# jhuggins/viabel

Measured on AMD Instinct MI355X. Metric: ELBO-gradient evals/sec (D=1024, N_mc=4096), higher is better.
Workload: dtype f64

## Files before the change

viabel_amd/csrc/vb_fullrank.hip:

```cpp
#include "vb_gemm_f64.h"
#include "vb_fit.h"

namespace vb {

constexpr double kLog2PiFr = 1.8378770664093454835606594728112;

__device__ __forceinline__ double fr_wave_sum(double x) {
#pragma unroll
  for (int off = 32; off > 0; off >>= 1) x += __shfl_down(x, off, 64);
  return x;
}

__device__ __forceinline__ double fr_block_sum(double x, double* sh) {
  x = fr_wave_sum(x);
  const int lane = threadIdx.x & 63, wave = threadIdx.x >> 6;
  __syncthreads();
  if (lane == 0) sh[wave] = x;
  __syncthreads();
  return (sh[0] + sh[1]) + (sh[2] + sh[3]);
}

__global__ void __launch_bounds__(256) fr_unpack_kernel(const double* __restrict__ theta, int d,
                                                        int64_t ldl, double* __restrict__ Lt,
                                                        double* __restrict__ mu, double* __restrict__ copy = nullptr) {
// ... 282 lines not shown
        if (roww) g[i] *= rw[i];
        if (square) g[i] *= g[i];
        if (!in) g[i] = (fr_d2){0.0, 0.0}, z[i] = (fr_d2){0.0, 0.0};
        if (!ok1) g[i].y = 0.0, z[i].y = 0.0;
        if (Gscaled && in) *reinterpret_cast<fr_d2*>(Gscaled + r * ldz + col) = g[i] * rs[i];
        s += g[i];
        if (fmode == 1) f = fma(hiv.x * g[i].x, g[i].x, fma(hiv.y * g[i].y, g[i].y, f));
        if (fmode == 2) f = fma(0.5 * z[i].x, g[i].x, fma(0.5 * z[i].y, g[i].y, f));
        if (fmode == 3) f = fma(-0.5 * scal * z[i].x, z[i].x, fma(-0.5 * scal * z[i].y, z[i].y, f));
      }
    }
  }
  cs[q][c] = s;
  __syncthreads();
  if (q == 0 && ok0) {
    const fr_d2 tot = (cs[0][c] + cs[1][c]) + (cs[2][c] + cs[3][c]);
    colpart[(int64_t)blockIdx.y * ldz + col] = tot.x;
    if (ok1) colpart[(int64_t)blockIdx.y * ldz + col + 1] = tot.y;
  }
  f = fr_block_sum(f, sh);
  if (threadIdx.x == 0) fpart[(int64_t)blockIdx.y * gridDim.x + blockIdx.x] = f;
}

__global__ void __launch_bounds__(256) fr_fold_msum_kernel(const double* __restrict__ Mpart, int msplits, int64_t slab,
                                                           int d, int64_t ldz, int k_split, int bm_rows,
                                                           double* __restrict__ Mout, int nb_b,
                                                           const double* __restrict__ P, int64_t ldp,
                                                           const double* __restrict__ mu,
                                                           const double* __restrict__ mean, double* __restrict__ b) {
  if ((int)blockIdx.x >= nb_b) {
    const int bpr = (int)((ldz / 2 + 255) / 256);
    const int blk = (int)blockIdx.x - nb_b, r = blk / bpr;
    const int cp = (blk - r * bpr) * 256 + (int)threadIdx.x;
    if (2 * cp >= ldz) return;
    const int64_t idx = (int64_t)r * ldz + 2 * cp;
    const int z0 = (r / bm_rows * bm_rows) / kGemmBK * kGemmBK / k_split;
    fr_d2 s = (fr_d2){0.0, 0.0};
    for (int zb = z0; zb < msplits; zb += 4) {
      fr_d2 v[4];
#pragma unroll
      for (int u = 0; u < 4; ++u)
        v[u] = *reinterpret_cast<const fr_d2*>(Mpart + (zb + u < msplits ? zb + u : msplits - 1) * slab + idx);
      s = zb == z0 ? v[0] : s + v[0];
#pragma unroll
      for (int u = 1; u < 4; ++u)
        if (zb + u < msplits) s += v[u];
    }
    *reinterpret_cast<fr_d2*>(Mout + idx) = s;
    return;
  }
  __shared__ fr_d2 part[64][4];
  const int p = threadIdx.x & 3, kg = threadIdx.x >> 2;
  const int col = (int)blockIdx.x * 8 + 2 * p;
  const int colc = col < d ? col : 0;
  const int kper = (d + 63) / 64;
  const int k0 = kg * kper, k1 = k0 + kper < d ? k0 + kper : d;
  fr_d2 s = (fr_d2){0.0, 0.0};
  for (int kb = k0; kb < k1; kb += 16) {
    fr_d2 v[16];
    double c[16];
#pragma unroll
    for (int u = 0; u < 16; ++u) {
      const int k = kb + u < k1 ? kb + u : k1 - 1;
      v[u] = *reinterpret_cast<const fr_d2*>(P + (int64_t)k * ldp + colc);
      c[u] = mu[k] - mean[k];
    }
#pragma unroll
    for (int u = 0; u < 16; ++u)
      if (kb + u < k1) s += v[u] * c[u];
  }
  part[kg][p] = s;
  __syncthreads();
  if (kg == 0) {
    fr_d2 tot = part[0][p];
#pragma unroll
    for (int q = 1; q < 64; ++q) tot += part[q][p];
    if (col < d) b[col] = tot.x;
    if (col + 1 < d) b[col + 1] = tot.y;
  }
}

static int fr_fold_splits(int d) {
  const int s = d / (16 * kGemmBK);
  return s < 1 ? 1 : (s > 8 ? 8 : s);
}

__global__ void __launch_bounds__(256) fr_fold_ssum_kernel(const double* __restrict__ Spart, int gsplits, int64_t slab, int d,
                                                           int64_t ldl, const double* __restrict__ colpart, int64_t ldz,
                                                           const double* __restrict__ M, const double* __restrict__ b,
                                                           double n_rows, int nb_cs, int nb_s,
                                                           double* __restrict__ S, double* __restrict__ svec,
                                                           double* __restrict__ csg) {
  if ((int)blockIdx.x < nb_cs) {
    __shared__ fr_d2 part[64][4];
    const int p = threadIdx.x & 3, kg = threadIdx.x >> 2;
    const int col = (int)blockIdx.x * 8 + 2 * p;
    const int colc = col < d ? col : 0;
    const int kper = (d + 63) / 64;
    const int k0 = kg * kper, k1 = k0 + kper < d ? k0 + kper : d;
    fr_d2 acc = (fr_d2){0.0, 0.0};
    for (int kb = k0; kb < k1; kb += 16) {
      fr_d2 v[16];
      double c[16];
#pragma unroll
      for (int u = 0; u < 16; ++u) {
        const int k = kb + u < k1 ? kb + u : k1 - 1;
        v[u] = *reinterpret_cast<const fr_d2*>(M + (int64_t)k * ldz + colc);
        c[u] = colpart[k];
      }
      for (int z = 1; z < gsplits; ++z)
#pragma unroll
        for (int u = 0; u < 16; ++u) c[u] += colpart[(int64_t)z * ldz + (kb + u < k1 ? kb + u : k1 - 1)];
#pragma unroll
      for (int u = 0; u < 16; ++u)
        if (kb + u < k1) acc += v[u] * c[u];
    }
    part[kg][p] = acc;
    __syncthreads();
    if (kg == 0) {
      fr_d2 tot = part[0][p];
#pragma unroll
      for (int q = 1; q < 64; ++q) tot += part[q][p];
      if (col < d) csg[col] = -tot.x - n_rows * b[col];
      if (col + 1 < d) csg[col + 1] = -tot.y - n_rows * b[col + 1];
    }
    return;
  }
  if ((int)blockIdx.x < nb_cs + nb_s) {
    const int k = ((int)blockIdx.x - nb_cs) * 256 + (int)threadIdx.x;
    if (k >= ldz) return;
    double s = 0.0;
    if (k < d) {
      s = colpart[k];
      for (int z = 1; z < gsplits; ++z) s += colpart[(int64_t)z * ldz + k];
    }
    svec[k] = s;
    return;
  }
  int bi = 0, bj = (int)blockIdx.x - nb_cs - nb_s;
  while (bj > bi) bj -= ++bi;
  __shared__ double tile[32][33];
  const int tx = threadIdx.x & 31, ty = threadIdx.x >> 5;
  const int i0 = bi * 32, j0 = bj * 32;
  double v[4];
  int64_t idx[4];
#pragma unroll
  for (int q = 0; q < 4; ++q) {
// ... 790 lines not shown
#endif
  *tiles2_out = (unsigned)n_p2;
  return VB_OK;
}


enum FrDense {
  kDenseNoG,
  kDenseCallerG,
  kDensePersistent,
  kDenseChain
};

struct FrRoute {
  bool mvt = false, pd = false, glm = false, source = false, overlap = false;
  int n_cu = 0;
  int64_t n = 0, d = 0, ldl = 0, ldz = 0, ldr = 0, slab = 0, pslab = 0, np = 0, glm_part = 0;
  int D = 0, n_rb = 0, cs_gx = 0, n_fpart = 0;
  int tri1 = 0, tri3 = 0;
  int splits = 1;
  int kparts = 1;
  unsigned sum_blocks = 0;
  bool fold_shape = false;
  int msplits = 1;
  bool fold = false;
  int csplits = 1;
  int cfgc = 0;
  int fz_mode = 0;
  FrDense dense = kDenseChain;
  bool model_ksplit = false;
  bool caller_z = false;
  bool fused_sums = false;
  bool diag_f = false;
  bool cs_only = false;
  bool g_prescaled = false;
  bool scale_rows_w = false;
  bool two_passes = false;
  bool colpass = false;
  bool colpass_keeps_f = false;
  int fmode = 0;
  bool grad_colsums = false;
  bool grad_launch = true;
  int cfg3 = 0;
  bool f_per_tile = false;
};

static FrRoute fr_route(const vb_ctx* ctx, const ModelDev& m, int64_t n, int64_t d, bool mvt, bool pd, bool row_scaled,
// ... 27 lines not shown
  if (r.splits > max_splits) r.splits = max_splits;
  if (r.splits < 1) r.splits = 1;
  r.n_rb = (int)((n + 127) / 128);
  r.cs_gx = (D + 127) / 128;
  r.glm_part = r.glm ? gemm_max_blocks(n, m.n_data) : 0;
  r.ldr = r.glm ? round_up(m.n_data, 16) : 0;
  r.n_fpart = funnel ? (int)((n + 3) / 4) : r.source ? (int)n : r.n_rb * r.cs_gx + (int)r.glm_part;

  const bool sums_in_gemms = !mvt && !wm.roww && !row_scaled && n % kGemmBK == 0 && gemm_uses_dma(s1) &&
                             (int64_t)r.splits <= r.n_rb;
  r.fused_sums = gauss_full && sums_in_gemms;
  r.diag_f = gauss_diag && sums_in_gemms;

  if (!row_scaled && !pd && !gauss_diag) {
    const long tiles64 = gemm_count_blocks(s1, 64, 64);
    if (tiles64 < 2L * n_cu && D >= 48 * kGemmBK) r.kparts = (int)((2L * n_cu + tiles64 - 1) / tiles64);
    if (r.kparts > 4) r.kparts = 4;
    while (r.kparts > 1 && (D % (kGemmBK * r.kparts) != 0 || D / r.kparts < 16 * kGemmBK)) --r.kparts;
    if ((int64_t)r.kparts * r.pslab > (int64_t)(r.splits + 1) * r.slab) r.kparts = 1;
  }
  r.sum_blocks = (unsigned)((r.pslab / 2 + 255) / 256);

  r.fold_shape = !mvt && gauss_full && !pd && d >= VB_FR_FOLD_MIN_D && n >= (int64_t)VB_FR_FOLD_MIN_ROWS_PER_D * d;
  r.msplits = fr_fold_splits(D);
  r.fold = r.fold_shape && r.fused_sums && r.kparts == 1 && !wm.z_ready && !wm.g_ready && n >= d + 2;

  r.fz_mode = ctx->fr_fused_mode;
  if (r.fz_mode < 0) {
    const char* e = getenv("VB_FR_FUSED");
    r.fz_mode = e ? atoi(e) : 0;
  }
  if (!(r.fused_sums && r.kparts == 1 && n % 128 == 0 && D % 64 == 0 && (int64_t)n * r.ldz * 8 < ((int64_t)1 << 31)))
    r.fz_mode = 0;
  if ((r.fz_mode != 2 && r.fz_mode != 3) || pd || r.fold || wm.g_ready) r.fz_mode = 0;
  r.dense = r.fold ? kDenseNoG : wm.g_ready ? kDenseCallerG : r.fz_mode >= 2 ? kDensePersistent : kDenseChain;
  r.model_ksplit = r.kparts > 1 && r.fused_sums;
  r.caller_z = wm.z_ready != nullptr && (funnel || r.source || r.glm);

  r.g_prescaled = funnel && wm.roww != nullptr;
  r.scale_rows_w = wm.roww != nullptr && !r.g_prescaled;
  r.cs_only = r.diag_f || (!r.fused_sums && !mvt && (funnel || r.source) && (!wm.roww || r.g_prescaled) && !row_scaled &&
                           n % kGemmBK == 0 && gemm_uses_dma(s3) && (int64_t)r.splits <= r.n_rb);
  const bool f_from_pass = !(funnel || r.source);
  r.colpass = !r.fused_sums && !r.cs_only;
  r.two_passes = pd && r.colpass && f_from_pass;
  r.colpass_keeps_f = f_from_pass && !r.two_passes;
  r.fmode = gauss_diag ? 1 : r.glm ? 3 : (gauss_full && !wm.g_ready) ? 2 : 0;

  r.grad_launch = r.fz_mode != 3;
  r.grad_colsums = r.fused_sums || r.cs_only;
  if (r.grad_launch && r.grad_colsums && gemm_count_blocks(s3, 128, 64) * r.splits * 100 >= 190L * n_cu) r.cfg3 = 2;
  r.f_per_tile = r.fused_sums || r.diag_f;
  if (r.fold) {
    r.csplits = fr_fold_csplits(D, n_cu, r.splits + 1);
    const GemmArgs sc = gemm_product(nullptr, 0, nullptr, 0, D, D, D, 2);
    if (gemm_count_blocks(sc, 64, 64) * r.csplits <= 4L * n_cu) r.cfgc = 4;
    else r.cfgc = gemm_count_blocks(sc, 128, 64) * r.csplits * 100 >= 190L * n_cu ? 2 : 3;
  }
  return r;
}

struct FrBufs {
  const double* E = nullptr;
  int64_t lde = 0;
  double *mu = nullptr, *Lt = nullptr;
  double *Z = nullptr, *G = nullptr, *Cpart = nullptr, *colpart = nullptr, *fpart = nullptr;
  double* Rm = nullptr;
  double *Mpart = nullptr, *bvec = nullptr;
  double *Sg = nullptr, *svec = nullptr, *csg = nullptr;
  double *Xa = nullptr, *T = nullptr, *sq = nullptr;
  FrSums S;
};

static int fr_carve(vb_ctx* ctx, const FrRoute& r, const NoiseSlot& ns, int set, FrBufs* out) {
  const int64_t n = r.n, ldz = r.ldz, slab = r.slab;
  int64_t off = 0;
  auto carve = [&off](int64_t doubles) {
    const int64_t o = off;
    off += round_up(doubles, 16);
    return o;
  };
  const int64_t o_mu = carve(ldz), o_lt = carve(slab), o_z = carve(n * ldz), o_g = carve(n * ldz),
                o_cpart = carve((int64_t)(r.splits + 1) * slab), o_col = carve((int64_t)(r.n_rb + 1) * ldz),
                o_fpart = carve((int64_t)r.n_fpart + (int64_t)r.n_rb * r.cs_gx + gemm_max_blocks(n, r.D) + (n * ldz) / 512 + 1),
                o_r = carve(r.glm ? n * r.ldr : 0);
  const int64_t o_mpart = r.fold_shape ? carve((int64_t)(r.msplits + 1) * slab) : 0, o_bvec = r.fold_shape ? carve(ldz) : 0;
  const int64_t o_xa = r.pd ? carve(slab) : 0, o_t = r.pd ? carve(slab) : 0, o_m2 = r.pd ? carve(256) : 0;
  FrBufs b;
  b.S.off_col = 16;
  b.S.off_c = 16 + ldz;
  b.S.len = 16 + ldz + (r.mvt ? slab : round_up(r.np, 16));
  const int64_t o_sums = carve(b.S.len * (r.overlap ? 2 : 1));
  VB_TRY(ensure(ctx, ctx->fr_work, (size_t)off * sizeof(double)));
  double* base = (double*)ctx->fr_work.ptr;
  b.E = (const double*)ns.buf.ptr;
  b.lde = ns.ld;
  b.mu = base + o_mu, b.Lt = base + o_lt, b.Z = base + o_z, b.G = base + o_g, b.Cpart = base + o_cpart;
  b.colpart = base + o_col, b.fpart = base + o_fpart, b.Rm = base + o_r;
  b.Mpart = base + o_mpart, b.bvec = base + o_bvec;
  if (r.fold) b.Sg = b.G, b.svec = b.G + slab, b.csg = b.G + slab + ldz;
  b.Xa = base + o_xa, b.T = base + o_t, b.sq = base + o_m2;
  b.S.sums = base + o_sums + (int64_t)set * b.S.len;
  *out = b;
  return VB_OK;
}

static int fr_stream_plan(vb_ctx* ctx, const FrRoute& r, int* set) {
  Pipeline& P = ctx->pipe;
  hipStream_t st = ctx->stream;
  *set = 0;
  if (r.overlap) {
    VB_TRY(pipe_init(ctx));
    *set = (int)(ctx->fr_seq++ & 1);
    if (P.fin_valid[*set]) VB_HIP(ctx, hipStreamWaitEvent(st, P.ev_fin[*set], 0));
  } else if (P.post_pending) {
    VB_HIP(ctx, hipStreamWaitEvent(st, P.ev_fin[P.last_set], 0));
    P.post_pending = false;
  }
  return VB_OK;
}

static int fr_prepare_mvt(vb_ctx* ctx, const FrRoute& r, const FrBufs& b, const double* mu_dev, const double* root_dev) {
// ... 69 lines not shown
static int fr_model_funnel(vb_ctx* ctx, const FrRoute& r, const FrBufs& b, const ModelDev& m, const double* Z,
                           const double* roww) {
  hipLaunchKernelGGL(fr_funnel_kernel, dim3((unsigned)((r.n + 3) / 4)), dim3(256), 0, ctx->stream, Z, b.G, r.ldz, r.n, r.D, m,
                     b.fpart, roww);
  return VB_OK;
}

static int fr_model_source(vb_ctx* ctx, const FrRoute& r, const FrBufs& b, const double* Z) {
  return model_rows_enqueue(ctx, ctx->stream, Z, r.ldz, r.n, r.D, b.G, r.ldz, b.fpart);
}

static int fr_model_glm(vb_ctx* ctx, const FrRoute& r, const FrBufs& b, const ModelDev& m, const double* Z) {
  hipStream_t st = ctx->stream;
  double* part = b.fpart + (int64_t)r.n_rb * r.cs_gx;
  VB_HIP(ctx, hipMemsetAsync(part, 0, (size_t)r.glm_part * sizeof(double), st));
  const GemmArgs gh = gemm_product(Z, r.ldz, m.p1, m.ldq, (int)r.n, (int)m.n_data, r.D, 0);
  gemm_f64_launch<true>(st, gh, 1, r.n_cu, EpiGlm{b.Rm, r.ldr, m.p2, part, m.link, m.aux});
  VB_HIP(ctx, hipGetLastError());
  return glm_grad_enqueue(ctx, st, m, b.Rm, r.ldr, Z, b.G, r.ldz, r.n, r.D);
}

static int fr_model_folded(vb_ctx* ctx, const FrRoute& r, const FrBufs& b, const ModelDev& m) {
  hipStream_t st = ctx->stream;
  const int D = r.D, msplits = r.msplits;
  double* Mres = msplits > 1 ? b.Mpart + (int64_t)msplits * r.slab : b.Mpart;
  const GemmArgs gm = gemm_product(b.Lt, r.ldl, m.p1, m.ldp, D, D, D, 4);
  gemm_f64_launch<true>(st, gm, msplits, r.n_cu, EpiSplitSlab{b.Mpart, r.ldz, r.slab}, 4);
  const int ks = (int)round_up((D + msplits - 1) / msplits, kGemmBK);
  const int nb_sum = msplits > 1 ? D * (int)((r.ldz / 2 + 255) / 256) : 0, nb_b = (D + 7) / 8;
  hipLaunchKernelGGL(fr_fold_msum_kernel, dim3((unsigned)(nb_sum + nb_b)), dim3(256), 0, st, (const double*)b.Mpart, msplits,
                     r.slab, D, r.ldz, ks, 64, Mres, nb_b, m.p1, (int64_t)m.ldp, (const double*)b.mu, m.p0, b.bvec);
  VB_HIP(ctx, hipGetLastError());
  return VB_OK;
}

static int fr_grad_folded(vb_ctx* ctx, const FrRoute& r, const FrBufs& b, unsigned* tiles3) {
  hipStream_t st = ctx->stream;
  const int D = r.D;
  const double* M = r.msplits > 1 ? b.Mpart + (int64_t)r.msplits * r.slab : b.Mpart;
  GemmArgs gs = gemm_product(b.E, b.lde, b.E, b.lde, D, D, (int)r.n, 2);
  prof_events(ctx, &gs.ev0, &gs.ev1, 1, VB_PROF_FR_GRAD_GEMM);
  if (r.cfg3 == 2) VB_TRY(tri2_tile_map(ctx, D, 128, 64, &gs.tile_map, &gs.tile_blocks));
  gemm_f64_launch<false>(st, gs, r.splits, r.n_cu, EpiSplitSlabCs{b.Cpart, r.ldl, r.slab, b.colpart, r.ldz}, r.cfg3);
  VB_HIP(ctx, hipGetLastError());
  const int nb_cs = (D + 7) / 8, nb_s = (int)((r.ldz + 255) / 256), tiles = (D + 31) / 32;
  hipLaunchKernelGGL(fr_fold_ssum_kernel, dim3((unsigned)(nb_cs + nb_s + tiles * (tiles + 1) / 2)), dim3(256), 0, st,
                     (const double*)b.Cpart, r.splits, r.slab, D, r.ldl, (const double*)b.colpart, r.ldz, M,
                     (const double*)b.bvec, (double)r.n, nb_cs, nb_s, b.Sg, b.svec, b.csg);
  VB_HIP(ctx, hipGetLastError());
  GemmArgs gc = gemm_product(M, r.ldz, b.Sg, r.ldl, D, D, D, 2);
  if (r.cfgc == 2) VB_TRY(tri2_tile_map(ctx, D, 128, 64, &gc.tile_map, &gc.tile_blocks));
  *tiles3 = gemm_f64_launch<false>(st, gc, r.csplits, r.n_cu,
                                   EpiFoldSlabF{b.Cpart, r.ldl, r.slab, b.bvec, b.svec, b.Lt, r.ldl, b.fpart}, r.cfgc);
  VB_HIP(ctx, hipGetLastError());
  return VB_OK;
}

static int fr_model_gauss_full(vb_ctx* ctx, const FrRoute& r, const FrBufs& b, const ModelDev& m, const double* row_scale,
                               const double* g_ready, double** G, unsigned* tiles2) {
  hipStream_t st = ctx->stream;
  const int D = r.D;
  *G = b.G;
  GemmArgs g2 = gemm_product(b.Z, r.ldz, m.p1, m.ldp, (int)r.n, D, D, 0);
  switch (r.dense) {
    case kDenseNoG:
      return fr_model_folded(ctx, r, b, m);
    case kDenseCallerG:
      *G = const_cast<double*>(g_ready);
      return VB_OK;
    case kDensePersistent: {
      const GemmArgs g1 = gemm_product(b.E, b.lde, b.Lt, r.ldl, (int)r.n, D, D, r.tri1);
// ... 24 lines not shown
                      double* fpart, const double* row_scale) {
  hipLaunchKernelGGL(fr_colsum_kernel, dim3((unsigned)r.cs_gx, (unsigned)r.n_rb), dim3(256), 0, ctx->stream, (const double*)G, Z,
                     r.ldz, r.n, r.D, fmode, m.p1, b.colpart, fpart, r.glm ? 1.0 / (m.tau * m.tau) : 0.0,
                     (const double*)nullptr, 0, row_scale ? G : (double*)nullptr, row_scale);
  VB_HIP(ctx, hipGetLastError());
  return VB_OK;
}

static int fr_rowscale(vb_ctx* ctx, const FrRoute& r, double* G, const double* w) {
  hipLaunchKernelGGL(fr_rowscale_kernel, dim3((unsigned)r.n, (unsigned)((r.D + 255) / 256)), dim3(256), 0, ctx->stream, G, r.ldz,
                     r.n, r.D, w);
  VB_HIP(ctx, hipGetLastError());
  return VB_OK;
}

static int fr_score(vb_ctx* ctx, const FrRoute& r, const FrBufs& b, const ModelDev& m, double* G, const double* Z) {
  if (r.two_passes) VB_TRY(fr_colpass(ctx, r, b, m, G, Z, r.fmode, b.fpart, nullptr));
  const GemmArgs gy = gemm_product(b.E, b.lde, b.T, r.ldl, (int)r.n, r.D, r.D, 3);
  gemm_f64_launch<true>(ctx->stream, gy, 1, r.n_cu, EpiAccumulate{G, r.ldz});
  VB_HIP(ctx, hipGetLastError());
  return VB_OK;
}

static int fr_grad_product(vb_ctx* ctx, const FrRoute& r, const FrBufs& b, const double* G, unsigned* tiles3) {
  hipStream_t st = ctx->stream;
  *tiles3 = 0;
  if (r.fold) return fr_grad_folded(ctx, r, b, tiles3);
  if (!r.grad_launch) return VB_OK;
  GemmArgs g3 = gemm_product(G, r.ldz, b.E, b.lde, r.D, r.D, (int)r.n, r.tri3);
  prof_events(ctx, &g3.ev0, &g3.ev1, 1, VB_PROF_FR_GRAD_GEMM);
  if (r.cfg3 == 2) VB_TRY(tri2_tile_map(ctx, r.D, 128, 64, &g3.tile_map, &g3.tile_blocks));
  if (r.grad_colsums)
    *tiles3 = gemm_f64_launch<false>(st, g3, r.splits, r.n_cu, EpiSplitSlabCs{b.Cpart, r.ldl, r.slab, b.colpart, r.ldz}, r.cfg3);
  else
    *tiles3 = gemm_f64_launch<false>(st, g3, r.splits, r.n_cu, EpiSplitSlab{b.Cpart, r.ldl, r.slab});
  VB_HIP(ctx, hipGetLastError());
  return VB_OK;
}

static int fr_finish_mvt(vb_ctx* ctx, const FrRoute& r, const FrBufs& b, FrSums* sums_out) {
  fr_reduce_launch(ctx, ctx->stream, (const double*)b.Cpart, r.splits, r.slab, r.D, r.ldl, (const double*)b.colpart, r.n_rb, r.ldz,
                   (const double*)b.fpart, r.n_fpart, b.S, 1, nullptr);
  VB_HIP(ctx, hipGetLastError());
  if (ctx->comm) VB_TRY(comm_allreduce_sum(ctx, ctx->stream, b.S.sums, (size_t)b.S.len));
  *sums_out = b.S;
  return VB_OK;
}

static int fr_finish_dense(vb_ctx* ctx, const FrRoute& r, const FrBufs& b, const ModelDev& m, int set, int n_fpart_red,
                           const double* theta_dev, double* out_dev, int64_t n_total, const FrWeighted& wm) {
// ... 74 lines not shown

  const double* Z = b.Z;
  double* G = b.G;
  unsigned tiles2 = 0, tiles3 = 0;
  if (m.id == VB_MODEL_GAUSS_DIAG) {
    tiles2 = fr_model_gauss_diag(ctx, r, b, m, row_scale);
  } else if (m.id == VB_MODEL_GAUSS_FULL) {
    VB_TRY(fr_model_gauss_full(ctx, r, b, m, row_scale, wm.g_ready, &G, &tiles2));
  } else {
    Z = fr_sample(ctx, r, b, nullptr, row_scale, wm.z_ready);
    VB_HIP(ctx, hipGetLastError());
    if (m.id == VB_MODEL_FUNNEL) VB_TRY(fr_model_funnel(ctx, r, b, m, Z, wm.roww));
    else if (r.source) VB_TRY(fr_model_source(ctx, r, b, Z));
    else VB_TRY(fr_model_glm(ctx, r, b, m, Z));
  }
  VB_HIP(ctx, hipGetLastError());

  if (r.scale_rows_w) VB_TRY(fr_rowscale(ctx, r, G, wm.roww));
  if (pd) VB_TRY(fr_score(ctx, r, b, m, G, Z));
  if (r.colpass)
    VB_TRY(fr_colpass(ctx, r, b, m, G, Z, r.two_passes ? 0 : r.fmode, r.colpass_keeps_f ? b.fpart : b.fpart + r.n_fpart,
                      row_scale));
  else if (row_scale) VB_TRY(fr_rowscale(ctx, r, G, row_scale));
  VB_TRY(fr_grad_product(ctx, r, b, G, &tiles3));

  if (mvt) return fr_finish_mvt(ctx, r, b, sums_out);
  const int n_fpart_red = r.fold ? (int)tiles3 * r.csplits : r.f_per_tile ? (int)tiles2 : r.n_fpart;
  return fr_finish_dense(ctx, r, b, m, set, n_fpart_red, theta_dev, out_dev, n_total, wm);
}

int fr_sample_enqueue(vb_ctx* ctx, const NoiseSlot& ns, int64_t n, int64_t d, const double* theta_dev, double* Z,
                      const double* mu_dev, const double* root_dev, const double* row_scale) {
  if (n <= 0 || d <= 0 || n > ns.n || d != ns.d) return fail(ctx, VB_ERR_INVALID, "noise slot shape mismatch");
  const int D = (int)d;
  const int64_t ldl = round_up(d, 16), ldz = ldl;
  hipStream_t st = ctx->stream;
  const double* E = (const double*)ns.buf.ptr;
  const int n_cu = ctx->prop.multiProcessorCount;
  if (theta_dev) {
    VB_TRY(ensure(ctx, ctx->fr_work, (size_t)(ldz + d * ldl) * sizeof(double)));
    double* mu = (double*)ctx->fr_work.ptr;
    double* Lt = mu + ldz;
    hipLaunchKernelGGL(fr_unpack_kernel, dim3((unsigned)((d + 31) / 32), (unsigned)((d + 31) / 32)), dim3(256), 0, st, theta_dev, D, ldl,
                       Lt, mu);
    gemm_f64_launch<true>(st, gemm_product(E, ns.ld, Lt, ldl, (int)n, D, D, 1), 1, n_cu, EpiStoreZ{Z, ldz, mu, nullptr, row_scale});
  } else {
    gemm_f64_launch<true>(st, gemm_product(E, ns.ld, root_dev, ldl, (int)n, D, D, 0), 1, n_cu,
// ... 14 lines not shown
```

viabel_amd/csrc/vb_gemm_f64.h:

```cpp
#pragma once

#include "vb_common.h"

#include <cstdlib>
#include <type_traits>
#include <utility>

namespace vb {

typedef double d2v __attribute__((ext_vector_type(2)));
typedef double d4v __attribute__((ext_vector_type(4)));

constexpr int kGemmBK = 16;

#ifdef VB_GEMM_CLOCK
__device__ long long vb_gemm_dbg[8 * 4096];
#endif

struct GemmArgs {
  const double* A = nullptr;
  const double* B = nullptr;
  int64_t lda = 0, ldb = 0;
  int M = 0, N = 0, K = 0;
  int tiles_m = 0, tiles_n = 0;
  int tri_mode = 0;
  int k_split = 0;
  int batch = 0;
  int64_t batch_a = 0, batch_b = 0;
  const int* tile_map = nullptr;
  int tile_blocks = 0;
  int tri4_splits = 0;
  int xcd_group = 0;
  int prio_div = 0;
  hipEvent_t ev0 = nullptr, ev1 = nullptr;
#ifdef VB_GEMM_CLOCK
  int dbg_bn_min = 0, dbg_bn_max = 1 << 30;
  int dbg_prio_slabs = 0;
#endif
};

inline GemmArgs gemm_product(const double* A, int64_t lda, const double* B, int64_t ldb, int M, int N, int K, int tri_mode) {
  GemmArgs g;
  g.A = A, g.lda = lda, g.B = B, g.ldb = ldb;
  g.M = M, g.N = N, g.K = K, g.tri_mode = tri_mode;
  return g;
}

template <class E, class = void>
struct EpiReduces : std::false_type {};
template <class E>
struct EpiReduces<E, std::void_t<decltype(std::declval<E>().part)>> : std::true_type {};

template <class E, class = void>
struct EpiPairs : std::false_type {};
// ... 225 lines not shown
#include "vb_gemm_f64_dma.h"

namespace vb {

inline int gemm_tiles(int x, int b) { return (x + b - 1) / b; }

inline int64_t gemm_max_blocks(int64_t M, int64_t N) { return ((M + 63) / 64) * ((N + 63) / 64); }

inline long gemm_count_blocks(const GemmArgs& g, int bm_rows, int bn_cols) {
  const int tm = gemm_tiles(g.M, bm_rows), tn = gemm_tiles(g.N, bn_cols);
  if (g.tri_mode != 2) return (long)tm * tn;
  long blocks = 0;
  for (int bm = 0; bm < tm; ++bm) {
    const int cnt = (bm * bm_rows + bm_rows - 1) / bn_cols + 1;
    blocks += cnt < tn ? cnt : tn;
  }
  return blocks;
}

inline bool gemm_uses_dma(const GemmArgs& g) {
  return g.K % kGemmBK == 0 && g.M > 0 && g.N > 0;
}

template <bool A_KCONTIG, class Epi>
inline unsigned gemm_f64_launch(hipStream_t st, GemmArgs g, int splits, int n_cu, const Epi& epi, int cfg = 0,
                                int flags = 0) {
  constexpr bool kNarrowOk = A_KCONTIG && !EpiColsum<Epi>::value;
  constexpr bool kNarrowAuto = kNarrowOk && !EpiReduces<Epi>::value && !EpiRowSums<Epi>::value;
  if (splits < 1) splits = 1;
  int ks = g.batch ? g.K : gemm_tiles(g.K, splits);
  g.k_split = gemm_tiles(ks, kGemmBK) * kGemmBK;
  const bool dma = gemm_uses_dma(g) && !(flags & 1);
  if (g.tri_mode == 3 && (!dma || splits != 1 || g.batch)) g.tri_mode = 0;
  if (g.tri_mode == 4 && (!dma || !A_KCONTIG || g.batch)) g.tri_mode = 0;
  if (cfg == 0) {
    if (dma && (g.tri_mode == 1 || g.tri_mode == 3) && splits == 1 && gemm_count_blocks(g, 128, 64) < 4L * n_cu) {
      cfg = 4;
      if (kNarrowAuto && !g.batch && gemm_count_blocks(g, 64, 64) <= 2L * n_cu) cfg = 8;
    } else if (dma && g.tri_mode == 0 && g.batch == 0 && gemm_count_blocks(g, 128, 128) * splits >= 2L * n_cu) {
      cfg = 6;
    } else if (!dma && gemm_count_blocks(g, 128, 128) * splits >= 2L * n_cu) {
      cfg = 1;
    } else if (gemm_count_blocks(g, 128, 64) * splits * 100 >= 190L * n_cu) {
      cfg = 2;
    } else {
      cfg = 3;
      if (kNarrowAuto && dma && g.tri_mode == 0 && !g.batch && gemm_count_blocks(g, 64, 64) * splits <= (long)n_cu) cfg = 7;
    }
  }
  if (!kNarrowOk && cfg >= 7) cfg = 4;
  if (!dma && cfg > 3) cfg = (cfg == 4 || cfg >= 7) ? 3 : cfg == 6 ? 1 : 2;
  const int bm_rows = (cfg == 3 || cfg == 4 || cfg >= 7) ? 64 : 128, bn_cols = cfg >= 7 ? 32 : (cfg == 1 || cfg == 6) ? 128 : 64;
  g.tiles_m = gemm_tiles(g.M, bm_rows);
  g.tiles_n = gemm_tiles(g.N, bn_cols);
  if (splits % 8 != 0 || g.batch) g.xcd_group = 0;
  dim3 grid(g.tile_map ? (unsigned)g.tile_blocks : (unsigned)gemm_count_blocks(g, bm_rows, bn_cols), 1, (unsigned)splits);
  if (g.tri_mode == 4 && splits > 1) {
    g.tri4_splits = splits;
    long items = 0;
    for (int bm = 0; bm < g.tiles_m; ++bm) items += (long)(splits - (bm * bm_rows / kGemmBK * kGemmBK) / g.k_split) * g.tiles_n;
    grid = dim3((unsigned)items, 1, 1);
  }
  g.prio_div = (g.tri_mode != 1 && g.tri_mode != 3 && g.tri_mode != 4) ? n_cu : 0;
  if (dma) {
    if (cfg == 1) gemm_f64_dma_launch<A_KCONTIG, 4, 16, 3, Epi>(st, g, grid, epi);
    else if (cfg == 2) gemm_f64_dma_launch<A_KCONTIG, 4, 8, 3, Epi>(st, g, grid, epi);
    else if (cfg == 3) gemm_f64_dma_launch<A_KCONTIG, 2, 8, 3, Epi>(st, g, grid, epi);
    else if (cfg == 4) gemm_f64_dma_launch<A_KCONTIG, 2, 8, 2, Epi>(st, g, grid, epi);
    else if (cfg == 6) gemm_f64_dma_launch<A_KCONTIG, 4, 16, 2, Epi>(st, g, grid, epi);
    else if (cfg >= 7) {
      if constexpr (kNarrowOk) {
        if (cfg == 7) gemm_f64_dma_launch<A_KCONTIG, 2, 4, 3, Epi>(st, g, grid, epi);
        else gemm_f64_dma_launch<A_KCONTIG, 2, 4, 2, Epi>(st, g, grid, epi);
      }
    }
    else gemm_f64_dma_launch<A_KCONTIG, 4, 8, 2, Epi>(st, g, grid, epi);
    return grid.x;
  }
  if (cfg == 1)
    hipExtLaunchKernelGGL((gemm_f64_kernel<A_KCONTIG, 4, 16, Epi>), grid, dim3(256), 0, st, g.ev0, g.ev1, 0, g, epi);
  else if (cfg == 2)
    hipExtLaunchKernelGGL((gemm_f64_kernel<A_KCONTIG, 4, 8, Epi>), grid, dim3(256), 0, st, g.ev0, g.ev1, 0, g, epi);
  else
    hipExtLaunchKernelGGL((gemm_f64_kernel<A_KCONTIG, 2, 8, Epi>), grid, dim3(256), 0, st, g.ev0, g.ev1, 0, g, epi);
  return grid.x;
}

}
```

viabel_amd/csrc/vb_gemm_f64_dma.h:

```cpp
#pragma once

namespace vb {

typedef __attribute__((address_space(1))) const void* gemm_gptr;
typedef __attribute__((address_space(3))) void* gemm_lptr;

struct GemmNoDep {
  static constexpr int kAuxA = 0;
  __device__ __forceinline__ void before_slab(int, int, int, bool) const {}
  __device__ __forceinline__ void publish(int, int, int) const {}
};

template <bool A_KCONTIG, int AF, int NB, int STAGES, class Epi, class Dep>
__device__ __forceinline__ void gemm_f64_dma_tile(const GemmArgs& g, const Epi& epi, const Dep& dep, const int bx,
                                                  const int bz_in, const int gx) {
  int bz = bz_in;
  constexpr int BM = 32 * AF, BN = 8 * NB;
  constexpr int kStages = STAGES;
  static_assert(STAGES == 2 || STAGES == 3, "two or three LDS stages");
  constexpr int kATile = BM * kGemmBK, kBTile = kGemmBK * BN;
  constexpr int kAUnits = kATile / 128, kBUnits = kBTile / 128;
  constexpr int UPW = (kAUnits + kBUnits) / 4;
  static_assert((kAUnits + kBUnits) % 4 == 0, "units must divide over the 4 waves");
  extern __shared__ double gemm_lds[];
  double* As = gemm_lds;
  double* Bs = gemm_lds + kStages * kATile;

  const int t = threadIdx.x;
  const int lane = t & 63, wave = __builtin_amdgcn_readfirstlane(t >> 6);
  const int wm = wave >> 1, wn = wave & 1;
#ifdef VB_GEMM_CLOCK
  const long long dbg_t0 = clock64(), dbg_w0 = wall_clock64();
  long long dbg_t1 = dbg_t0, dbg_t2 = dbg_t0;
#endif

  double local = 0.0;
  int bm, bn;
  if (g.tri_mode == 2 && g.tile_map) {
    bm = g.tile_map[2 * bx];
// ... 2 lines not shown
      if constexpr (EpiReduces<Epi>::value)
        if (t == 0) epi.part[(int64_t)bz * gx + bx] = 0.0;
      return;
    }
  } else if (g.tri_mode == 2) {
    int idx = bx;
    bm = 0;
    for (;;) {
      const int cnt = min(g.tiles_n, (bm * BM + BM - 1) / BN + 1);
      if (idx < cnt) break;
      idx -= cnt;
      ++bm;
    }
    bn = idx;
  } else if (g.tri_mode == 1 || g.tri_mode == 3) {
    const int tn = g.tiles_n;
    const int idx = bx / g.tiles_m, half = (tn + 1) / 2;
    bn = idx < half ? tn - 1 - idx : idx - half;
    if (g.tri_mode == 3) bn = g.tiles_n - 1 - bn;
    bm = bx % g.tiles_m;
#ifdef VB_GEMM_CLOCK
    if (bn < g.dbg_bn_min || bn > g.dbg_bn_max) return;
#endif
  } else if (g.tri_mode == 4 && g.tri4_splits > 1) {
    int idx = bx;
    bm = 0;
    int z0 = 0;
    for (;;) {
      z0 = (bm * BM / kGemmBK * kGemmBK) / g.k_split;
      const int cnt = (g.tri4_splits - z0) * g.tiles_n;
      if (idx < cnt || bm == g.tiles_m - 1) break;
      idx -= cnt;
      ++bm;
    }
    bz = z0 + idx / g.tiles_n;
    bn = idx % g.tiles_n;
  } else if (g.tri_mode == 4) {
    bm = bx / g.tiles_n;
    bn = bx % g.tiles_n;
  } else {
    bn = bx / g.tiles_m;
    bm = bx % g.tiles_m;
  }
  const int m0 = bm * BM, n0 = bn * BN;
  int k_begin = g.batch ? 0 : bz * g.k_split;
  int k_end = (g.batch || k_begin + g.k_split >= g.K) ? g.K : k_begin + g.k_split;
  if (g.tri_mode == 3) {
    const int kmin = n0 / kGemmBK * kGemmBK;
    if (k_begin < kmin) k_begin = kmin < k_end ? kmin : k_end;
  }
  if (g.tri_mode == 4) {
    const int kmin = m0 / kGemmBK * kGemmBK;
    if (k_begin < kmin) k_begin = kmin < k_end ? kmin : k_end;
  }
  const double* __restrict__ gA = g.A + (g.batch ? (int64_t)bz * g.batch_a : 0);
  const double* __restrict__ gB = g.B + (g.batch ? (int64_t)bz * g.batch_b : 0);
  if (g.tri_mode == 1) {
    const int kmax = n0 + BN;
    if (k_end > kmax) k_end = kmax;
// ... 348 lines not shown
    gemm_f64_dma_kernel(const GemmArgs g, const Epi epi) {
  int bx = (int)blockIdx.x, bz = (int)blockIdx.z;
  if (g.xcd_group) {
    const unsigned lin = blockIdx.x + gridDim.x * blockIdx.z, slot = lin >> 3;
    bz = (int)((lin & 7) + 8 * (slot / gridDim.x));
    bx = (int)(slot % gridDim.x);
  }
  gemm_f64_dma_tile<A_KCONTIG, AF, NB, STAGES, Epi, GemmNoDep>(g, epi, GemmNoDep{}, bx, bz, (int)gridDim.x);
}

template <bool A_KCONTIG, int AF, int NB, int STAGES, class Epi>
inline void gemm_f64_dma_launch(hipStream_t st, const GemmArgs& g, dim3 grid, const Epi& epi) {
  constexpr size_t lds = (size_t)STAGES * (32 * AF * kGemmBK + kGemmBK * 8 * NB) * sizeof(double);
  static bool configured = false;
  if (!configured) {
    (void)hipFuncSetAttribute(reinterpret_cast<const void*>(&gemm_f64_dma_kernel<A_KCONTIG, AF, NB, STAGES, Epi>),
                              hipFuncAttributeMaxDynamicSharedMemorySize, (int)lds);
    configured = true;
  }
  hipExtLaunchKernelGGL((gemm_f64_dma_kernel<A_KCONTIG, AF, NB, STAGES, Epi>), grid, dim3(256), lds, st, g.ev0, g.ev1,
                        0, g, epi);
}

}
```

Baseline: 5563.

## Replace split-K triangular model GEMM with paired row-block kernel; fold b into ssum

The folded model GEMM (L^T times P, triangular mode 4) no longer uses split-K partial slabs plus a separate summation kernel. A new paired kernel instead lets each block process a row block and its mirror, which balances the triangular work without partial buffers. The b = P·(mu-mean) reduction moves from the removed msum kernel into the ssum kernel, saving one launch and the Mpart traffic. In exchange there is less parallelism per GEMM (no K split) and the ssum kernel now does extra serial work per block.

```diff
diff --git a/viabel_amd/csrc/vb_fullrank.hip b/viabel_amd/csrc/vb_fullrank.hip
--- a/viabel_amd/csrc/vb_fullrank.hip
+++ b/viabel_amd/csrc/vb_fullrank.hip
@@ -328,83 +328,34 @@
   if (threadIdx.x == 0) fpart[(int64_t)blockIdx.y * gridDim.x + blockIdx.x] = f;
 }
 
-__global__ void __launch_bounds__(256) fr_fold_msum_kernel(const double* __restrict__ Mpart, int msplits, int64_t slab,
-                                                           int d, int64_t ldz, int k_split, int bm_rows,
-                                                           double* __restrict__ Mout, int nb_b,
-                                                           const double* __restrict__ P, int64_t ldp,
-                                                           const double* __restrict__ mu,
-                                                           const double* __restrict__ mean, double* __restrict__ b) {
-  if ((int)blockIdx.x >= nb_b) {
-    const int bpr = (int)((ldz / 2 + 255) / 256);
-    const int blk = (int)blockIdx.x - nb_b, r = blk / bpr;
-    const int cp = (blk - r * bpr) * 256 + (int)threadIdx.x;
-    if (2 * cp >= ldz) return;
-    const int64_t idx = (int64_t)r * ldz + 2 * cp;
-    const int z0 = (r / bm_rows * bm_rows) / kGemmBK * kGemmBK / k_split;
-    fr_d2 s = (fr_d2){0.0, 0.0};
-    for (int zb = z0; zb < msplits; zb += 4) {
-      fr_d2 v[4];
-#pragma unroll
-      for (int u = 0; u < 4; ++u)
-        v[u] = *reinterpret_cast<const fr_d2*>(Mpart + (zb + u < msplits ? zb + u : msplits - 1) * slab + idx);
-      s = zb == z0 ? v[0] : s + v[0];
-#pragma unroll
-      for (int u = 1; u < 4; ++u)
-        if (zb + u < msplits) s += v[u];
-    }
-    *reinterpret_cast<fr_d2*>(Mout + idx) = s;
-    return;
-  }
-  __shared__ fr_d2 part[64][4];
-  const int p = threadIdx.x & 3, kg = threadIdx.x >> 2;
-  const int col = (int)blockIdx.x * 8 + 2 * p;
-  const int colc = col < d ? col : 0;
-  const int kper = (d + 63) / 64;
-  const int k0 = kg * kper, k1 = k0 + kper < d ? k0 + kper : d;
-  fr_d2 s = (fr_d2){0.0, 0.0};
-  for (int kb = k0; kb < k1; kb += 16) {
-    fr_d2 v[16];
-    double c[16];
-#pragma unroll
-    for (int u = 0; u < 16; ++u) {
-      const int k = kb + u < k1 ? kb + u : k1 - 1;
-      v[u] = *reinterpret_cast<const fr_d2*>(P + (int64_t)k * ldp + colc);
-      c[u] = mu[k] - mean[k];
-    }
-#pragma unroll
-    for (int u = 0; u < 16; ++u)
-      if (kb + u < k1) s += v[u] * c[u];
-  }
-  part[kg][p] = s;
-  __syncthreads();
-  if (kg == 0) {
-    fr_d2 tot = part[0][p];
-#pragma unroll
-    for (int q = 1; q < 64; ++q) tot += part[q][p];
-    if (col < d) b[col] = tot.x;
-    if (col + 1 < d) b[col + 1] = tot.y;
-  }
-}
-
-static int fr_fold_splits(int d) {
-  const int s = d / (16 * kGemmBK);
-  return s < 1 ? 1 : (s > 8 ? 8 : s);
-}
-
 __global__ void __launch_bounds__(256) fr_fold_ssum_kernel(const double* __restrict__ Spart, int gsplits, int64_t slab, int d,
                                                            int64_t ldl, const double* __restrict__ colpart, int64_t ldz,
-                                                           const double* __restrict__ M, const double* __restrict__ b,
-                                                           double n_rows, int nb_cs, int nb_s,
-                                                           double* __restrict__ S, double* __restrict__ svec,
-                                                           double* __restrict__ csg) {
+                                                           const double* __restrict__ M, const double* __restrict__ P,
+                                                           int64_t ldp, const double* __restrict__ mu,
+                                                           const double* __restrict__ mean, double n_rows, int nb_cs,
+                                                           int nb_s, double* __restrict__ S, double* __restrict__ svec,
+                                                           double* __restrict__ b, double* __restrict__ csg) {
   if ((int)blockIdx.x < nb_cs) {
-    __shared__ fr_d2 part[64][4];
+    __shared__ fr_d2 part[2][64][4];
     const int p = threadIdx.x & 3, kg = threadIdx.x >> 2;
     const int col = (int)blockIdx.x * 8 + 2 * p;
     const int colc = col < d ? col : 0;
     const int kper = (d + 63) / 64;
     const int k0 = kg * kper, k1 = k0 + kper < d ? k0 + kper : d;
-    fr_d2 acc = (fr_d2){0.0, 0.0};
+    fr_d2 acc = (fr_d2){0.0, 0.0}, bacc = (fr_d2){0.0, 0.0};
+    for (int kb = k0; kb < k1; kb += 16) {
+      fr_d2 v[16];
+      double c[16];
+#pragma unroll
+      for (int u = 0; u < 16; ++u) {
+        const int k = kb + u < k1 ? kb + u : k1 - 1;
+        v[u] = *reinterpret_cast<const fr_d2*>(P + (int64_t)k * ldp + colc);
+        c[u] = mu[k] - mean[k];
+      }
+#pragma unroll
+      for (int u = 0; u < 16; ++u)
+        if (kb + u < k1) bacc += v[u] * c[u];
+    }
     for (int kb = k0; kb < k1; kb += 16) {
       fr_d2 v[16];
       double c[16];
@@ -421,14 +372,15 @@
       for (int u = 0; u < 16; ++u)
         if (kb + u < k1) acc += v[u] * c[u];
     }
-    part[kg][p] = acc;
+    part[0][kg][p] = acc;
+    part[1][kg][p] = bacc;
     __syncthreads();
     if (kg == 0) {
-      fr_d2 tot = part[0][p];
-#pragma unroll
-      for (int q = 1; q < 64; ++q) tot += part[q][p];
-      if (col < d) csg[col] = -tot.x - n_rows * b[col];
-      if (col + 1 < d) csg[col + 1] = -tot.y - n_rows * b[col + 1];
+      fr_d2 tot = part[0][0][p], btot = part[1][0][p];
+#pragma unroll 16
+      for (int q = 1; q < 64; ++q) tot += part[0][q][p], btot += part[1][q][p];
+      if (col < d) b[col] = btot.x, csg[col] = -tot.x - n_rows * btot.x;
+      if (col + 1 < d) b[col + 1] = btot.y, csg[col + 1] = -tot.y - n_rows * btot.y;
     }
     return;
   }
@@ -1265,7 +1217,6 @@
   int kparts = 1;
   unsigned sum_blocks = 0;
   bool fold_shape = false;
-  int msplits = 1;
   bool fold = false;
   int csplits = 1;
   int cfgc = 0;
@@ -1339,7 +1290,6 @@
   r.sum_blocks = (unsigned)((r.pslab / 2 + 255) / 256);
 
   r.fold_shape = !mvt && gauss_full && !pd && d >= VB_FR_FOLD_MIN_D && n >= (int64_t)VB_FR_FOLD_MIN_ROWS_PER_D * d;
-  r.msplits = fr_fold_splits(D);
   r.fold = r.fold_shape && r.fused_sums && r.kparts == 1 && !wm.z_ready && !wm.g_ready && n >= d + 2;
 
   r.fz_mode = ctx->fr_fused_mode;
@@ -1383,7 +1333,7 @@
   double *mu = nullptr, *Lt = nullptr;
   double *Z = nullptr, *G = nullptr, *Cpart = nullptr, *colpart = nullptr, *fpart = nullptr;
   double* Rm = nullptr;
-  double *Mpart = nullptr, *bvec = nullptr;
+  double *Mf = nullptr, *bvec = nullptr;
   double *Sg = nullptr, *svec = nullptr, *csg = nullptr;
   double *Xa = nullptr, *T = nullptr, *sq = nullptr;
   FrSums S;
@@ -1401,7 +1351,7 @@
                 o_cpart = carve((int64_t)(r.splits + 1) * slab), o_col = carve((int64_t)(r.n_rb + 1) * ldz),
                 o_fpart = carve((int64_t)r.n_fpart + (int64_t)r.n_rb * r.cs_gx + gemm_max_blocks(n, r.D) + (n * ldz) / 512 + 1),
                 o_r = carve(r.glm ? n * r.ldr : 0);
-  const int64_t o_mpart = r.fold_shape ? carve((int64_t)(r.msplits + 1) * slab) : 0, o_bvec = r.fold_shape ? carve(ldz) : 0;
+  const int64_t o_mf = r.fold_shape ? carve(slab) : 0, o_bvec = r.fold_shape ? carve(ldz) : 0;
   const int64_t o_xa = r.pd ? carve(slab) : 0, o_t = r.pd ? carve(slab) : 0, o_m2 = r.pd ? carve(256) : 0;
   FrBufs b;
   b.S.off_col = 16;
@@ -1414,7 +1364,7 @@
   b.lde = ns.ld;
   b.mu = base + o_mu, b.Lt = base + o_lt, b.Z = base + o_z, b.G = base + o_g, b.Cpart = base + o_cpart;
   b.colpart = base + o_col, b.fpart = base + o_fpart, b.Rm = base + o_r;
-  b.Mpart = base + o_mpart, b.bvec = base + o_bvec;
+  b.Mf = base + o_mf, b.bvec = base + o_bvec;
   if (r.fold) b.Sg = b.G, b.svec = b.G + slab, b.csg = b.G + slab + ldz;
   b.Xa = base + o_xa, b.T = base + o_t, b.sq = base + o_m2;
   b.S.sums = base + o_sums + (int64_t)set * b.S.len;
@@ -1530,22 +1480,17 @@
 
 static int fr_model_folded(vb_ctx* ctx, const FrRoute& r, const FrBufs& b, const ModelDev& m) {
   hipStream_t st = ctx->stream;
-  const int D = r.D, msplits = r.msplits;
-  double* Mres = msplits > 1 ? b.Mpart + (int64_t)msplits * r.slab : b.Mpart;
+  const int D = r.D;
   const GemmArgs gm = gemm_product(b.Lt, r.ldl, m.p1, m.ldp, D, D, D, 4);
-  gemm_f64_launch<true>(st, gm, msplits, r.n_cu, EpiSplitSlab{b.Mpart, r.ldz, r.slab}, 4);
-  const int ks = (int)round_up((D + msplits - 1) / msplits, kGemmBK);
-  const int nb_sum = msplits > 1 ? D * (int)((r.ldz / 2 + 255) / 256) : 0, nb_b = (D + 7) / 8;
-  hipLaunchKernelGGL(fr_fold_msum_kernel, dim3((unsigned)(nb_sum + nb_b)), dim3(256), 0, st, (const double*)b.Mpart, msplits,
-                     r.slab, D, r.ldz, ks, 64, Mres, nb_b, m.p1, (int64_t)m.ldp, (const double*)b.mu, m.p0, b.bvec);
-  VB_HIP(ctx, hipGetLastError());
-  return VB_OK;
-}
-
-static int fr_grad_folded(vb_ctx* ctx, const FrRoute& r, const FrBufs& b, unsigned* tiles3) {
+  gemm_f64_launch<true, true>(st, gm, 1, r.n_cu, EpiSplitSlab{b.Mf, r.ldz, r.slab});
+  VB_HIP(ctx, hipGetLastError());
+  return VB_OK;
+}
+
+static int fr_grad_folded(vb_ctx* ctx, const FrRoute& r, const FrBufs& b, const ModelDev& m, unsigned* tiles3) {
   hipStream_t st = ctx->stream;
   const int D = r.D;
-  const double* M = r.msplits > 1 ? b.Mpart + (int64_t)r.msplits * r.slab : b.Mpart;
+  const double* M = b.Mf;
   GemmArgs gs = gemm_product(b.E, b.lde, b.E, b.lde, D, D, (int)r.n, 2);
   prof_events(ctx, &gs.ev0, &gs.ev1, 1, VB_PROF_FR_GRAD_GEMM);
   if (r.cfg3 == 2) VB_TRY(tri2_tile_map(ctx, D, 128, 64, &gs.tile_map, &gs.tile_blocks));
@@ -1553,8 +1498,8 @@
   VB_HIP(ctx, hipGetLastError());
   const int nb_cs = (D + 7) / 8, nb_s = (int)((r.ldz + 255) / 256), tiles = (D + 31) / 32;
   hipLaunchKernelGGL(fr_fold_ssum_kernel, dim3((unsigned)(nb_cs + nb_s + tiles * (tiles + 1) / 2)), dim3(256), 0, st,
-                     (const double*)b.Cpart, r.splits, r.slab, D, r.ldl, (const double*)b.colpart, r.ldz, M,
-                     (const double*)b.bvec, (double)r.n, nb_cs, nb_s, b.Sg, b.svec, b.csg);
+                     (const double*)b.Cpart, r.splits, r.slab, D, r.ldl, (const double*)b.colpart, r.ldz, M, m.p1,
+                     (int64_t)m.ldp, (const double*)b.mu, m.p0, (double)r.n, nb_cs, nb_s, b.Sg, b.svec, b.bvec, b.csg);
   VB_HIP(ctx, hipGetLastError());
   GemmArgs gc = gemm_product(M, r.ldz, b.Sg, r.ldl, D, D, D, 2);
   if (r.cfgc == 2) VB_TRY(tri2_tile_map(ctx, D, 128, 64, &gc.tile_map, &gc.tile_blocks));
@@ -1625,10 +1570,11 @@
   return VB_OK;
 }
 
-static int fr_grad_product(vb_ctx* ctx, const FrRoute& r, const FrBufs& b, const double* G, unsigned* tiles3) {
+static int fr_grad_product(vb_ctx* ctx, const FrRoute& r, const FrBufs& b, const ModelDev& m, const double* G,
+                           unsigned* tiles3) {
   hipStream_t st = ctx->stream;
   *tiles3 = 0;
-  if (r.fold) return fr_grad_folded(ctx, r, b, tiles3);
+  if (r.fold) return fr_grad_folded(ctx, r, b, m, tiles3);
   if (!r.grad_launch) return VB_OK;
   GemmArgs g3 = gemm_product(G, r.ldz, b.E, b.lde, r.D, r.D, (int)r.n, r.tri3);
   prof_events(ctx, &g3.ev0, &g3.ev1, 1, VB_PROF_FR_GRAD_GEMM);
@@ -1749,7 +1695,7 @@
     VB_TRY(fr_colpass(ctx, r, b, m, G, Z, r.two_passes ? 0 : r.fmode, r.colpass_keeps_f ? b.fpart : b.fpart + r.n_fpart,
                       row_scale));
   else if (row_scale) VB_TRY(fr_rowscale(ctx, r, G, row_scale));
-  VB_TRY(fr_grad_product(ctx, r, b, G, &tiles3));
+  VB_TRY(fr_grad_product(ctx, r, b, m, G, &tiles3));
 
   if (mvt) return fr_finish_mvt(ctx, r, b, sums_out);
   const int n_fpart_red = r.fold ? (int)tiles3 * r.csplits : r.f_per_tile ? (int)tiles2 : r.n_fpart;
diff --git a/viabel_amd/csrc/vb_gemm_f64.h b/viabel_amd/csrc/vb_gemm_f64.h
--- a/viabel_amd/csrc/vb_gemm_f64.h
+++ b/viabel_amd/csrc/vb_gemm_f64.h
@@ -29,7 +29,6 @@
   int64_t batch_a = 0, batch_b = 0;
   const int* tile_map = nullptr;
   int tile_blocks = 0;
-  int tri4_splits = 0;
   int xcd_group = 0;
   int prio_div = 0;
   hipEvent_t ev0 = nullptr, ev1 = nullptr;
@@ -301,7 +300,7 @@
   return g.K % kGemmBK == 0 && g.M > 0 && g.N > 0;
 }
 
-template <bool A_KCONTIG, class Epi>
+template <bool A_KCONTIG, bool TRI4_PAIRS = false, class Epi>
 inline unsigned gemm_f64_launch(hipStream_t st, GemmArgs g, int splits, int n_cu, const Epi& epi, int cfg = 0,
                                 int flags = 0) {
   constexpr bool kNarrowOk = A_KCONTIG && !EpiColsum<Epi>::value;
@@ -327,6 +326,9 @@
       if (kNarrowAuto && dma && g.tri_mode == 0 && !g.batch && gemm_count_blocks(g, 64, 64) * splits <= (long)n_cu) cfg = 7;
     }
   }
+  static_assert(!TRI4_PAIRS || kNarrowAuto, "paired row blocks: A[m][k], an epilogue that only stores");
+  const bool pairs = TRI4_PAIRS && g.tri_mode == 4 && splits == 1;
+  if (pairs) cfg = 7;
   if (!kNarrowOk && cfg >= 7) cfg = 4;
   if (!dma && cfg > 3) cfg = (cfg == 4 || cfg >= 7) ? 3 : cfg == 6 ? 1 : 2;
   const int bm_rows = (cfg == 3 || cfg == 4 || cfg >= 7) ? 64 : 128, bn_cols = cfg >= 7 ? 32 : (cfg == 1 || cfg == 6) ? 128 : 64;
@@ -334,12 +336,7 @@
   g.tiles_n = gemm_tiles(g.N, bn_cols);
   if (splits % 8 != 0 || g.batch) g.xcd_group = 0;
   dim3 grid(g.tile_map ? (unsigned)g.tile_blocks : (unsigned)gemm_count_blocks(g, bm_rows, bn_cols), 1, (unsigned)splits);
-  if (g.tri_mode == 4 && splits > 1) {
-    g.tri4_splits = splits;
-    long items = 0;
-    for (int bm = 0; bm < g.tiles_m; ++bm) items += (long)(splits - (bm * bm_rows / kGemmBK * kGemmBK) / g.k_split) * g.tiles_n;
-    grid = dim3((unsigned)items, 1, 1);
-  }
+  if (pairs) grid = dim3((unsigned)((g.tiles_m + 1) / 2 * g.tiles_n), 1, 1);
   g.prio_div = (g.tri_mode != 1 && g.tri_mode != 3 && g.tri_mode != 4) ? n_cu : 0;
   if (dma) {
     if (cfg == 1) gemm_f64_dma_launch<A_KCONTIG, 4, 16, 3, Epi>(st, g, grid, epi);
@@ -348,6 +345,12 @@
     else if (cfg == 4) gemm_f64_dma_launch<A_KCONTIG, 2, 8, 2, Epi>(st, g, grid, epi);
     else if (cfg == 6) gemm_f64_dma_launch<A_KCONTIG, 4, 16, 2, Epi>(st, g, grid, epi);
     else if (cfg >= 7) {
+      if constexpr (TRI4_PAIRS) {
+        if (pairs) {
+          gemm_f64_dma_pair_launch<2, 4, 3, Epi>(st, g, grid, epi);
+          return grid.x;
+        }
+      }
       if constexpr (kNarrowOk) {
         if (cfg == 7) gemm_f64_dma_launch<A_KCONTIG, 2, 4, 3, Epi>(st, g, grid, epi);
         else gemm_f64_dma_launch<A_KCONTIG, 2, 4, 2, Epi>(st, g, grid, epi);
diff --git a/viabel_amd/csrc/vb_gemm_f64_dma.h b/viabel_amd/csrc/vb_gemm_f64_dma.h
--- a/viabel_amd/csrc/vb_gemm_f64_dma.h
+++ b/viabel_amd/csrc/vb_gemm_f64_dma.h
@@ -13,8 +13,7 @@
 
 template <bool A_KCONTIG, int AF, int NB, int STAGES, class Epi, class Dep>
 __device__ __forceinline__ void gemm_f64_dma_tile(const GemmArgs& g, const Epi& epi, const Dep& dep, const int bx,
-                                                  const int bz_in, const int gx) {
-  int bz = bz_in;
+                                                  const int bz, const int gx) {
   constexpr int BM = 32 * AF, BN = 8 * NB;
   constexpr int kStages = STAGES;
   static_assert(STAGES == 2 || STAGES == 3, "two or three LDS stages");
@@ -63,19 +62,6 @@
 #ifdef VB_GEMM_CLOCK
     if (bn < g.dbg_bn_min || bn > g.dbg_bn_max) return;
 #endif
-  } else if (g.tri_mode == 4 && g.tri4_splits > 1) {
-    int idx = bx;
-    bm = 0;
-    int z0 = 0;
-    for (;;) {
-      z0 = (bm * BM / kGemmBK * kGemmBK) / g.k_split;
-      const int cnt = (g.tri4_splits - z0) * g.tiles_n;
-      if (idx < cnt || bm == g.tiles_m - 1) break;
-      idx -= cnt;
-      ++bm;
-    }
-    bz = z0 + idx / g.tiles_n;
-    bn = idx % g.tiles_n;
   } else if (g.tri_mode == 4) {
     bm = bx / g.tiles_n;
     bn = bx % g.tiles_n;
@@ -470,4 +456,37 @@
                         0, g, epi);
 }
 
-}
+struct GemmPairNoDep : GemmNoDep {};
+
+template <int AF, int NB, int STAGES, class Epi>
+__global__ void __launch_bounds__(256, AF * NB > 32 ? (STAGES > 2 ? 1 : 2) : (AF * NB > 16 || STAGES > 2 ? 2 : 4))
+    gemm_f64_dma_pair_kernel(const GemmArgs g, const Epi epi) {
+  static_assert(!EpiReduces<Epi>::value && !EpiColsum<Epi>::value && !EpiRowSums<Epi>::value,
+                "the epilogue between the passes must leave LDS alone");
+  const int pair = (int)blockIdx.x / g.tiles_n, bn = (int)blockIdx.x % g.tiles_n;
+  const int mirror = g.tiles_m - 1 - pair;
+  const int passes = mirror > pair ? 2 : 1;
+#pragma unroll 1
+  for (int pass = 0; pass < passes; ++pass) {
+    const int bm = pass == 0 ? pair : mirror;
+    const int bx = bm * g.tiles_n + bn, bz = 0;
+    gemm_f64_dma_tile<true, AF, NB, STAGES, Epi, GemmPairNoDep>(g, epi, GemmPairNoDep{}, bx, bz, (int)gridDim.x);
+    __asm__ volatile("" ::: "memory");
+    __builtin_amdgcn_s_waitcnt(0);
+    __asm__ volatile("" ::: "memory");
+  }
+}
+
+template <int AF, int NB, int STAGES, class Epi>
+inline void gemm_f64_dma_pair_launch(hipStream_t st, const GemmArgs& g, dim3 grid, const Epi& epi) {
+  constexpr size_t lds = (size_t)STAGES * (32 * AF * kGemmBK + kGemmBK * 8 * NB) * sizeof(double);
+  static bool configured = false;
+  if (!configured) {
+    (void)hipFuncSetAttribute(reinterpret_cast<const void*>(&gemm_f64_dma_pair_kernel<AF, NB, STAGES, Epi>),
+                              hipFuncAttributeMaxDynamicSharedMemorySize, (int)lds);
+    configured = true;
+  }
+  hipExtLaunchKernelGGL((gemm_f64_dma_pair_kernel<AF, NB, STAGES, Epi>), grid, dim3(256), lds, st, g.ev0, g.ev1, 0, g, epi);
+}
+
+}
```

New measurement: 5713, median of 6. 2.7% higher.
